# UtkarshSaxena1/CiM_Quantization

Measured on AMD Instinct MI355X. Metric: quantized-MAC/s + fwd+bwd ms per ResNet-20 w3a3 CiM layer, batch 256, higher is better.
Workload: dtype i8+f32; 1 GPU; resnet20_w3a3_all_19_cim_convs_fwd_bwd_sgd; global_batch=256, per_gpu_batch=256, xbar=128, first_layer=w8a8, parallelism=dp1, exchange_segments=1, launch=hip_graph, recompute_psum=False

## Files before the change

### cim_quantization_amd/csrc/cimq_gx5.hip

```cpp
#include "cimq_bwd_dev.h"
#include "cimq_operands.h"

namespace cimq {

__global__ void prep_wg5_kernel(Geo g, const float* __restrict__ w_q, const float* __restrict__ sw_p, int total,
                                v4i* __restrict__ wg5) {
  const WSrc ws{w_q, *sw_p, 0, 0.f, 0.f};
  for (int t = blockIdx.x * blockDim.x + threadIdx.x; t < total; t += gridDim.x * blockDim.x) wg5_item(g, ws, wg5, t);
}

template <int CBN>
__device__ __forceinline__ void gx5_body(int bid, int nblk, const Geo& g, const X5& v, const uint32_t* __restrict__ st,
                                         const v4i* __restrict__ wg5, const Params& pp, const float* __restrict__ sw_p,
                                         const float* __restrict__ sa_p, const float* __restrict__ gout,
                                         const float* __restrict__ x, float* __restrict__ gx,
                                         float* __restrict__ gsa_part) {
  extern __shared__ __attribute__((aligned(16))) uint8_t smem[];
  const int WP = g.W + 2;
  const int PLANE = 6 * WP * 96;
  const int OW5 = 3 * PLANE + 32;
  constexpr int NW5 = 9 * 2 * CBN * 64;
  constexpr int NWI = (NW5 + 511) / 512;
  float* cel = reinterpret_cast<float*>(smem + OW5 + NW5 * 16);
  float* red = cel + 16;
  const int lane = threadIdx.x & 63, wave = threadIdx.x >> 6;
  const int r16 = lane & 15, g4 = lane >> 4;
  const float sw = *sw_p, sa = *sa_p;
  for (int t = threadIdx.x; t < 9; t += blockDim.x) cel[t] = pp.ckj[9 + t];
  if (threadIdx.x < 2) reinterpret_cast<uint4*>(smem + 3 * PLANE)[threadIdx.x] = make_uint4(0u, 0u, 0u, 0u);
  for (int t = threadIdx.x; t < 3 * 6 * 2 * 6; t += blockDim.x) {
    const int q = t % 6, rc = t / 6, side = rc & 1, pr = rc >> 1;
    reinterpret_cast<uint4*>(smem + (size_t)pr * WP * 96 + (side ? (WP - 1) * 96 : 0))[q] = make_uint4(0u, 0u, 0u, 0u);
  }
  __syncthreads();
  const bool std_mask =
      __builtin_amdgcn_ballot_w64(lane < 9 && cel[lane < 9 ? lane : 0] != (float)(1 << (lane / 3))) == 0ull;
  const float scale = sw / 3.f;
  const float inv_sa = 1.f / sa;
  float gpart = 0.f;
  const int cb = wave / v.NPG, pg = wave - cb * v.NPG;
  const int gpr = g.W >> 4;
  const int rl = pg / gpr, iw0 = 16 * (pg - rl * gpr);
  const int c_lo = 16 * cb, c_hi = 16 * cb + 15;
  const int gstride = g.onchw ? g.P : 1;

  const int NG = 6 * g.W * 4;
  for (int mt = bid; mt < v.nmt; mt += nblk) {
    const int b = mt / v.tpi, r0 = (mt - b * v.tpi) * 4;
    v4f acc = v4f{0.f, 0.f, 0.f, 0.f};
    float gvr[2][2][4];
#pragma unroll
    for (int hh = 0; hh < 2; ++hh)
#pragma unroll
      for (int k = 0; k < 2; ++k) {
        const int it = threadIdx.x + k * (int)blockDim.x;
        const int oq = (it & 3) + 4 * hh, rc = it >> 2, col = rc & (g.W - 1), row = rc >> v.lw;
        const int oh = r0 - 1 + row;
#pragma unroll
        for (int e = 0; e < 4; ++e) gvr[hh][k][e] = 0.f;
        if (hh < CBN && it < NG && (unsigned)oh < (unsigned)g.Ho) {
          const int pimg = oh * g.Wo + col;
          const int go = g.onchw ? (b * g.O + 4 * oq) * g.P + pimg : (b * g.P + pimg) * g.O + 4 * oq;
#pragma unroll
          for (int e = 0; e < 4; ++e) gvr[hh][k][e] = gout[go + e * gstride];
        }
      }
    for (int i = 0; i < g.T; ++i)
#pragma unroll
    for (int h = 0; h < 2; ++h) {
      if (h >= CBN) break;
      const int ih2 = i * CBN + h;
      v4i wv[NWI];
#pragma unroll
      for (int u = 0; u < NWI; ++u) {
        const int idx = threadIdx.x + u * 512;
        if (idx < NW5) wv[u] = wg5[ih2 * NW5 + idx];
      }
      uint4 s4r[2];
#pragma unroll
      for (int kk = 0; kk < 2; ++kk) {
        const int it = threadIdx.x + kk * 512;
        const int rc = it >> 2, col = rc & (g.W - 1), row = rc >> v.lw;
        const int oh = r0 - 1 + row;
        s4r[kk] = make_uint4(0u, 0u, 0u, 0u);
        if (it < NG && (unsigned)oh < (unsigned)g.Ho) {
          const int m = b * g.P + oh * g.Wo + col;
          s4r[kk] = *reinterpret_cast<const uint4*>(st + ((i * g.M + m) * g.O + 4 * ((it & 3) + 4 * h)));
        }
      }
      __syncthreads();
#pragma unroll
      for (int u = 0; u < NWI; ++u) {
        const int idx = threadIdx.x + u * 512;
        if (idx < NW5) reinterpret_cast<v4i*>(smem + OW5)[idx] = wv[u];
      }
      auto build = [&](auto stdc) {
        constexpr bool STD = decltype(stdc)::value;
#pragma unroll
        for (int kk = 0; kk < 2; ++kk) {
          const int it = threadIdx.x + kk * (int)blockDim.x;
          if (it >= NG) continue;
          const int oq = (it & 3) + 4 * h, rc = it >> 2, col = rc & (g.W - 1), row = rc >> v.lw;
          const float* gv = gvr[h][kk];
          const uint4 s4 = s4r[kk];
          const uint32_t sv[4] = {s4.x, s4.y, s4.z, s4.w};
          uint8_t* px = smem + (row * WP + col + 1) * 96 + 8 * (oq - 4 * h);
#pragma unroll
          for (int k = 0; k < 3; ++k) {
            float Gv[4];
#pragma unroll
            for (int e = 0; e < 4; ++e) {
              float E;
              if constexpr (STD) {
                E = (float)(__popc(sv[e] & pass_mask_k(k, 3)) << k);
              } else {
                E = 0.f;
#pragma unroll
                for (int j = 0; j < 3; ++j) E += ((sv[e] >> (3 * (k * 3 + j))) & 1u) ? cel[k * 3 + j] : 0.f;
              }
              Gv[e] = gv[e] * E;
            }
            uint32_t ph[2], pm[2], plo[2];
#pragma unroll
            for (int u = 0; u < 2; ++u) split3_pk(Gv[2 * u], Gv[2 * u + 1], ph[u], pm[u], plo[u]);
            *reinterpret_cast<uint2*>(px + 32 * k) = make_uint2(ph[0], ph[1]);
            *reinterpret_cast<uint2*>(px + PLANE + 32 * k) = make_uint2(pm[0], pm[1]);
            *reinterpret_cast<uint2*>(px + 2 * PLANE + 32 * k) = make_uint2(plo[0], plo[1]);
          }
        }
      };
      if (std_mask) build(std::true_type{});
      else build(std::false_type{});
      __syncthreads();
      if (9 * c_hi + 8 < i * g.xbar || 9 * c_lo >= (i + 1) * g.xbar) continue;
      const v4i* wb = reinterpret_cast<const v4i*>(smem + OW5) + cb * 64 + lane;
#pragma unroll
      for (int p = 0; p < 9; ++p) {
        const int kh = p / 3, kw = p - 3 * kh;
        const uint8_t* pa = smem + (size_t)((rl + 2 - kh) * WP + iw0 + r16 + 2 - kw) * 96 + 16 * g4;
#pragma unroll
        for (int s = 0; s < 2; ++s) {
          const v8bf ah = as_v8bf(*reinterpret_cast<const v4i*>(pa + 64 * s));
          const v8bf am = as_v8bf(*reinterpret_cast<const v4i*>(pa + PLANE + 64 * s));
          const v8bf al = as_v8bf(*reinterpret_cast<const v4i*>(pa + 2 * PLANE + 64 * s));
          const v8bf w = as_v8bf(wb[(p * 2 + s) * CBN * 64]);
          acc = __builtin_amdgcn_mfma_f32_16x16x32_bf16(ah, w, acc, 0, 0, 0);
          acc = __builtin_amdgcn_mfma_f32_16x16x32_bf16(am, w, acc, 0, 0, 0);
          acc = __builtin_amdgcn_mfma_f32_16x16x32_bf16(al, w, acc, 0, 0, 0);
        }
      }
    }
    const int ih = r0 + rl, iw = iw0 + 4 * g4;
    const int gi = ((b * g.C + c_lo + r16) * g.H + ih) * g.W + iw;
    const float4 xv4 = *reinterpret_cast<const float4*>(x + gi);
    const float xv[4] = {xv4.x, xv4.y, xv4.z, xv4.w};
    float o4[4];
#pragma unroll
    for (int r = 0; r < 4; ++r) {
      const float gqv = acc[r] * scale;
      const float y1 = xv[r] / sa;
      const float clv = clamp_nan(y1, 0.f, g.lsq_qp);
      const float rr2 = rintf(clv);
      const float rp = (rr2 - clv) + clv;
      const bool pass = (y1 >= 0.f) && (y1 <= g.lsq_qp);
      const float gy = pass ? gqv * sa : 0.f;
      o4[r] = pass ? gqv : 0.f;
      gpart += gqv * rp;
      gpart += -(gy * (y1 * inv_sa));
    }
    *reinterpret_cast<float4*>(gx + gi) = make_float4(o4[0], o4[1], o4[2], o4[3]);
  }
  for (int o = 32; o > 0; o >>= 1) gpart += __shfl_xor(gpart, o);
  __syncthreads();
  if (lane == 0) red[wave] = gpart;
  __syncthreads();
  if (threadIdx.x == 0) {
    float t = 0.f;
    for (int w = 0; w < 8; ++w) t += red[w];
    gsa_part[bid] = t;
  }
}

template <int CBN>
__global__ __attribute__((amdgpu_flat_work_group_size(512, 512), amdgpu_waves_per_eu(4, 8)))
void cim_bwd_gx5_kernel(Geo g, X5 v, const uint32_t* __restrict__ st, const v4i* __restrict__ wg5, Params pp,
                        const float* __restrict__ sw_p, const float* __restrict__ sa_p,
                        const float* __restrict__ gout, const float* __restrict__ x, float* __restrict__ gx,
                        float* __restrict__ gsa_part) {
  gx5_body<CBN>((int)blockIdx.x, (int)gridDim.x, g, v, st, wg5, pp, sw_p, sa_p, gout, x, gx, gsa_part);
}

}
```

### cim_quantization_amd/csrc/cimq_host.h

```cpp
#pragma once
#include <math.h>
#include <stdarg.h>
#include <stdio.h>
#include <string.h>

#include <algorithm>
#include <array>
#include <map>
#include <mutex>
#include <string>

#include "../../include/cimq.h"
#include "cimq_types.h"

namespace cimq {

inline thread_local std::string g_last_error;

inline int fail(int code, const char* fmt, ...) {
  char buf[512];
  va_list ap;
  va_start(ap, fmt);
  vsnprintf(buf, sizeof(buf), fmt, ap);
  va_end(ap);
// ... 538 lines not shown
  return g.input_kind == CIMQ_INPUT_RAW_LSQ && g.NBP == 4 && adc_ok && g.W % 4 == 0 &&
         g.P % 64 == 0 && g.lsq_qp >= 0.f && g.lsq_qp < 255.f && v3_plan(g).ok && (v7_bwd(g) || v7_w44_eval(g)) &&
         !c1_plan(g).ok;
}

struct Plan5 {
  bool ok;
  F5 v;
  size_t lds;
  int nob;
};

inline Plan5 f5_plan_compute(const Geo& g) {
  Plan5 p;
  memset(&p, 0, sizeof(p));
  if (tune("FWD5", 1) == 0) return p;
  if (!fwd_actq_ok(g) || g.mode != ADC_TERNARY || g.variant != VAR_LIBRARY) return p;
  if (g.nbw != 3 || g.nba != 3 || g.bsw != 1 || g.bsa != 1) return p;
  if (g.KH != 3 || g.KW != 3 || g.PH != 1 || g.PW != 1 || g.SH != g.SW || (g.SH != 1 && g.SH != 2)) return p;
  if (g.C % 16 != 0 || g.O % 16 != 0 || g.W % 4 != 0 || g.P % 16 != 0) return p;
  if (g.P >= 128 ? g.P % 128 != 0 : 128 % g.P != 0) return p;
  if (g.M % 128 != 0) return p;
  if (g.Wo % 16 != 0 && 16 % g.Wo != 0) return p;
  F5& v = p.v;
  v.lwo = 0;
  while ((1 << v.lwo) < g.Wo) ++v.lwo;
  if ((1 << v.lwo) != g.Wo) return p;
  v.lwi = 0;
  while ((1 << v.lwi) < g.W) ++v.lwi;
  if ((1 << v.lwi) != g.W) return p;
  if ((long long)g.Nin >= (1LL << 31) || (long long)g.T * g.M * g.O >= (1LL << 31) || (long long)g.M * g.O >= (1LL << 31))
    return p;
  const int PI = std::min(g.P, 128);
  v.IPM = 128 / PI;
  v.R = PI / g.Wo;
  v.RH = (v.R - 1) * g.SH + 3;
  v.WP = g.W + 2;
  v.nmt = g.M / 128;
  v.ntc = 0;
  for (int i = 0; i < g.T; ++i) {
    v.tc0[i] = (unsigned char)v.ntc;
    const int flo = i * g.xbar, fhi = std::min(flo + g.xbar, g.K);
    const int cblo = (flo / 9) / 16, cbhi = ((fhi - 1) / 9) / 16;
    for (int cb = cblo; cb <= cbhi; ++cb) {
      if (v.ntc >= kF5MaxTc) return p;
      v.tcb[v.ntc++] = (unsigned char)cb;
    }
  }
  v.tc0[g.T] = (unsigned char)v.ntc;
  p.nob = (g.OB16 % 2 == 0 && tune("FWD5_NOB2", 1)) ? 2 : 1;
  const size_t fixed = (size_t)p.nob * g.T * 9 * 16 * (16 + 4) + a16((size_t)2 * ((int)g.lsq_qp + 2) * 4) + 16;
  const size_t budget = (size_t)(p.nob == 2 ? tune("FWD5_LDS2_KB", 150) : tune("FWD5_LDS_KB", 80)) * 1024;
  auto need = [&](int tcm, int ncb) {
    return fixed + (size_t)p.nob * tcm * 9 * 1024 + (size_t)v.IPM * v.RH * ncb * v.WP * 48;
  };
  v.ngrp = 0;
  v.tcmax = 0;
  v.NCBP = 0;
  for (int i = 0; i < g.T;) {
    if (v.ngrp >= kF5MaxGrp) return p;
    int e = i + 1;
    auto span = [&](int a, int b) { return v.tcb[v.tc0[b] - 1] - v.tcb[v.tc0[a]] + 1; };
    auto pairs = [&](int a, int b) { return v.tc0[b] - v.tc0[a]; };
    if (need(std::max(v.tcmax, pairs(i, e)), std::max(v.NCBP, span(i, e))) > budget) return p;
    while (e < g.T && need(std::max(v.tcmax, pairs(i, e + 1)), std::max(v.NCBP, span(i, e + 1))) <= budget) ++e;
    const int q = v.ngrp++;
    v.gt0[q] = (unsigned char)i;
    v.gcb0[q] = v.tcb[v.tc0[i]];
    v.gcb1[q] = v.tcb[v.tc0[e] - 1];
    v.gown[q] = (unsigned char)(q == 0 ? v.gcb0[0] : v.gcb1[q - 1] + 1);
    v.tcmax = std::max(v.tcmax, pairs(i, e));
    v.NCBP = std::max(v.NCBP, span(i, e));
    i = e;
  }
  v.gt0[v.ngrp] = (unsigned char)g.T;
  p.lds = need(v.tcmax, v.NCBP);
  p.ok = p.lds <= budget;
  return p;
}
inline Plan5 f5_plan(const Geo& g) { return memo_geo<Plan5, f5_plan_compute>(g); }
inline size_t f5_frag_items(const Geo& g, const Plan5& p) { return p.ok ? (size_t)g.OB16 * p.v.ntc * 9 * 64 : 0; }
inline size_t f5_frag_bytes(const Geo& g) { return f5_frag_items(g, f5_plan(g)) * 16; }

struct PlanG5 {
  bool ok;
  G5 v;
  size_t lds;
  int pairs;
};

inline PlanG5 g5_plan_compute(const Geo& g) {
  PlanG5 p;
  memset(&p, 0, sizeof(p));
  if (tune("GW5", 1) == 0) return p;
  if (!v7_bwd(g) || g.variant != VAR_LIBRARY || g.NBP != 4 || g.nbw != 3 || g.nba != 3 || g.bsa != 1) return p;
  if (g.KH != 3 || g.KW != 3 || g.SH != g.SW || (g.SH != 1 && g.SH != 2) || g.PH != 1 || g.PW != 1 ||
      g.xbar != 128)
    return p;
  if (g.W != g.Wo * g.SH || g.H != g.Ho * g.SH) return p;
  if (g.SH == 2 && tune("GW5_S2", 1) == 0) return p;
  if (g.C % 16 != 0 || g.O % 16 != 0 || g.Wo % 4 != 0) return p;
  if (g.P >= 128 ? g.P % 128 != 0 : (128 % g.P != 0 || g.P % 16 != 0)) return p;
  if (g.M % 128 != 0) return p;
  if (g.T != (9 * g.C + 127) / 128) return p;
  G5& v = p.v;
  v.lwo = 0;
  while ((1 << v.lwo) < g.Wo) ++v.lwo;
  if ((1 << v.lwo) != g.Wo || 128 % g.Wo != 0) return p;
  v.lwi = v.lwo + (g.SH == 2 ? 1 : 0);
  if ((long long)g.Nin >= (1LL << 31)) return p;
  v.IPM = 128 / std::min(g.P, 128);
  v.R = std::min(g.P, 128) / g.Wo;
  v.RH = (v.R - 1) * g.SH + 3;
  v.WP = g.W + 2;
  if ((long long)16 * v.IPM * v.RH * v.WP >= (1LL << 16)) return p;
  if (g.SH == 1 && 16 * v.IPM * v.RH * g.W > 6 * 512) return p;
  v.nmt = g.M / 128;
  p.pairs = (g.C / 16) * g.OB16;
  const int want = std::max(1, tune("GW5_BLOCKS", 512) / p.pairs);
  v.nst = std::max(1, (v.nmt + want - 1) / want);
  v.nchunks = (v.nmt + v.nst - 1) / v.nst;
  p.lds = std::max((size_t)16 * v.IPM * v.RH * v.WP * 8, (size_t)3 * 8 * 64 * 16) + 64 + 4 * 260;
  p.ok = p.lds <= (size_t)80 * 1024;
  return p;
}
inline PlanG5 g5_plan(const Geo& g) { return memo_geo<PlanG5, g5_plan_compute>(g); }

struct PlanX5 {
  bool ok;
  X5 v;
  size_t lds;
  int nblk;
};

inline PlanX5 x5_plan_compute(const Geo& g) {
  PlanX5 p;
  memset(&p, 0, sizeof(p));
  if (tune("GX5", 1) == 0) return p;
  if (!v7_bwd(g) || g.variant != VAR_LIBRARY || g.NBP != 4 || g.nbw != 3 || g.nba != 3 || g.bsw != 1) return p;
  if (g.input_kind != CIMQ_INPUT_RAW_LSQ) return p;
  if (g.KH != 3 || g.KW != 3 || g.SH != 1 || g.SW != 1 || g.PH != 1 || g.PW != 1 || g.xbar != 128) return p;
  const bool c16 = g.C == 16 && g.O == 16 && g.W == 32, c32 = g.C == 32 && g.O == 32 && g.W == 16;
  if (!(c16 || c32) || g.H % 4 != 0 || g.Wo != g.W || g.Ho != g.H || g.T != (9 * g.C + 127) / 128) return p;
  p.v.tpi = g.H / 4;
  p.v.nmt = g.B * p.v.tpi;
  p.v.CBN = g.C / 16;
  p.v.NPG = g.W / 4;
  if (p.v.NPG * p.v.CBN != 8) return p;
  p.v.lw = g.W == 32 ? 5 : 4;
  if (6 * g.W * 4 > 2 * 512) return p;
  if ((long long)g.T * g.M * g.O >= (1LL << 31) || (long long)g.Nin >= (1LL << 31) || (long long)g.M * g.O >= (1LL << 31))
    return p;
  p.nblk = std::min(p.v.nmt, tune("GX5_GRID", 256));
  p.lds = (size_t)3 * 6 * (g.W + 2) * 96 + 32 + (size_t)9 * 2 * p.v.CBN * 1024 + 32 * 4;
  p.ok = p.lds <= (size_t)80 * 1024;
  return p;
}
inline PlanX5 x5_plan(const Geo& g) { return memo_geo<PlanX5, x5_plan_compute>(g); }
inline size_t x5_frag_bytes(const Geo& g) {
  const PlanX5 p = x5_plan(g);
  return p.ok ? (size_t)g.T * p.v.CBN * 9 * 2 * p.v.CBN * 64 * 16 : 0;
}

struct PlanR6 {
  bool ok;
  R6 v;
  size_t lds;
};

inline PlanR6 r6_plan_compute(const Geo& g) {
  PlanR6 p;
  memset(&p, 0, sizeof(p));
  if (!g.recompute || tune("R6", 1) == 0) return p;
  const Plan5 p5 = f5_plan(g);
  if (!p5.ok || !v7_bwd(g) || g.variant != VAR_LIBRARY || g.mode != ADC_TERNARY) return p;
  if (g.input_kind != CIMQ_INPUT_RAW_LSQ || g.nbw != 3 || g.nba != 3 || g.bsw != 1 || g.bsa != 1) return p;
  if (g.KH != 3 || g.KW != 3 || g.SH != 1 || g.SW != 1 || g.PH != 1 || g.PW != 1 || g.xbar != 128) return p;
  if (g.C != kR6C || g.O != kR6C || g.W != kR6W || g.Wo != g.W || g.Ho != g.H || g.H % kR6R != 0) return p;
  if (g.T != kR6T || g.lsq_qp >= 255.f || (long long)g.Nin >= (1LL << 31)) return p;
  if (p5.v.ntc != kR6T || p5.v.tc0[0] != 0 || p5.v.tc0[1] != 1 || p5.v.tc0[2] != 2) return p;
  for (int i = 0; i <= kR6T; ++i) p.v.tc0[i] = p5.v.tc0[i];
  p.v.ntc = p5.v.ntc;
  p.v.nmt = g.H / kR6R;
  p.lds = R6L::LDS;
  p.ok = true;
  return p;
}
inline PlanR6 r6_plan(const Geo& g) { return memo_geo<PlanR6, r6_plan_compute>(g); }
inline size_t r6_frag_bytes(const Geo& g) { return r6_plan(g).ok ? (size_t)kR6WxItems * 16 : 0; }


enum StateFmt {
  ST_NONE,
  ST_PERK,
  ST_V7,
  ST_V7X2,
  ST_PLANES,
  ST_C1,
  ST_DENSE,
};

struct Route {
  int fwd, gx, gw;
  bool actq;
  StateFmt state;
  int cst;
  FwdState fst;
  size_t st_bytes;
  bool codes;
  bool lsq_fused;
  int act_parts;
  int nchunks_bwd;
  int nchunks_ws;
  bool gw_own;
  bool gxw5;
  bool shift_stats;
  bool wgx, wcy, wg5, wx6;
};

inline Route route_compute(const Geo& g) {
  Route r;
  memset(&r, 0, sizeof(r));
  const bool raw = g.input_kind == CIMQ_INPUT_RAW_LSQ, v7b = v7_bwd(g), dense = dense_plan(g);
  r.actq = fwd_actq_ok(g) && (g.onchw || g.inference);
  r.fwd = v3_plan(g).ok ? ((g.onchw && r.actq && f5_plan(g).ok) ? CIMQ_ROUTE_FWD5 : CIMQ_ROUTE_V3)
        : dense         ? CIMQ_ROUTE_DENSE
                        : CIMQ_ROUTE_GENERAL;
  int nchunks, rows;
  gw_chunks(g, &rows, &nchunks);
  const int gen_parts = std::min(cdiv(g.Nin, 256), kLsqParts);
  r.act_parts = gen_parts;
  if (v7b) {
    r.lsq_fused = raw;
    r.nchunks_bwd = r.act_parts = g.B;
    if (g.onchw && !g.inference && r6_plan(g).ok) {
      r.gx = r.gw = CIMQ_ROUTE_R6;
    } else if (c1_plan(g).ok) {
      r.gx = r.gw = CIMQ_ROUTE_C1;
    } else if (v9_plan(g).ok) {
      r.gx = r.gw = CIMQ_ROUTE_FUSED;
    } else {
      const Plan7 p7 = v7_plan(g);
      const PlanX5 px = x5_plan(g);
      const PlanG5 pg = g5_plan(g);
      r.gx = px.ok ? CIMQ_ROUTE_GX5 : CIMQ_ROUTE_V7;
      r.gw = pg.ok ? CIMQ_ROUTE_GW5 : CIMQ_ROUTE_V7;
      r.act_parts = px.ok ? px.nblk : g.B * p7.v.nbands;
      r.nchunks_bwd = pg.ok ? pg.v.nchunks : p7.v.nchunks;
      r.gw_own = g.variant == VAR_LIBRARY;
      r.gxw5 = px.ok && pg.ok && tune("GXW5", 1);
    }
    if (!r.lsq_fused) r.act_parts = gen_parts;
  } else if (dense) {
    r.gx = r.gw = CIMQ_ROUTE_DENSE;
    r.lsq_fused = raw && dense_lsq_parts(g) > 0;
    if (r.lsq_fused) r.act_parts = dense_lsq_parts(g);
    r.nchunks_bwd = cdiv(g.M, dense_rows_per_chunk(g));
  } else {
    r.gx = r.gw = CIMQ_ROUTE_GENERAL;
    r.nchunks_bwd = nchunks;
  }
  r.nchunks_ws = std::max({nchunks, r.nchunks_bwd, r6_plan(g).ok ? g.B : 0});
  r.shift_stats = v7b && g.variant != VAR_LIBRARY;
  const StateFmt fam = dense                 ? ST_DENSE
                     : !v7_plan(g).ok        ? ST_PERK
                     : r.gx == CIMQ_ROUTE_C1 ? ST_C1
                     : g.NBP == 8            ? ST_PLANES
                     : g.nbw == 4            ? ST_V7X2
                                             : ST_V7;
  r.state = r.gx == CIMQ_ROUTE_R6 ? ST_NONE : fam;
  r.cst = (fam == ST_V7 || fam == ST_V7X2) ? g.nbw : (fam == ST_PLANES || fam == ST_C1) ? 8 : 0;
  r.fst = fam == ST_C1 ? FwdState::RECOMPUTE : FwdState::WRITE;
  r.st_bytes = r.state == ST_NONE ? (size_t)0
                                  : std::max({(size_t)g.T * g.nbw * g.M * g.O * (g.NBP == 4 ? 2 : 4),
                                              (size_t)g.T * g.M * g.O * (g.NBP == 4 ? 4 : 24),
                                              dense ? (size_t)g.T * g.M * g.O * 8 : (size_t)0});
  r.codes = r.fwd == CIMQ_ROUTE_FWD5 && r.gw == CIMQ_ROUTE_GW5;
  r.wgx = !v7b;
  r.wcy = v7b;
  r.wg5 = x5_plan(g).ok;
  r.wx6 = r6_plan(g).ok;
  if (g.inference) {
    r.gx = r.gw = CIMQ_ROUTE_NONE;
    r.state = ST_NONE;
    r.st_bytes = 0;
    if (v7_w44_eval(g)) r.cst = 4;
    if (r.cst != 0 && r.fst == FwdState::WRITE) r.fst = FwdState::NONE;
    r.codes = r.lsq_fused = r.gw_own = r.gxw5 = r.wgx = r.wcy = r.wg5 = r.wx6 = false;
  }
  return r;
}
inline Route route_of(const Geo& g) { return memo_geo<Route, route_compute>(g); }

inline FwdMode fwd_mode_of(const Geo& g, const Epi* ep) {
  if (!ep) return g.inference ? FwdMode::INFER : FwdMode::TRAIN;
  return ep->rvw1 ? FwdMode::VIEW : (ep->xq || ep->oq) ? FwdMode::CODES : FwdMode::EPI;
}

inline Geo module_form(Geo g) {
  g.onchw = v3_plan(g).ok ? 1 : 0;
  return g;
}

struct CtxLayout {
  size_t xcode, xhat, alut, wfrag, wf5, wg5, wx6, wgx, wcy, thi, tlo, mlo, mhi, coef, alpha, beta, bsum, ckj, flags, st;
  size_t lsq_scal;
  size_t wbytes;
// ... 250 lines not shown
```

### cim_quantization_amd/csrc/cimq_operands.h

```cpp
#pragma once
#include "cimq_device.h"

namespace cimq {

__device__ inline void pack_word(int8_t (&v)[8], int nbp, uint8_t* dst, long long idx) {
  uint32_t lo = (uint8_t)v[0] | ((uint32_t)(uint8_t)v[1] << 8) | ((uint32_t)(uint8_t)v[2] << 16) |
                ((uint32_t)(uint8_t)v[3] << 24);
  if (nbp == 4) {
    reinterpret_cast<uint32_t*>(dst)[idx] = lo;
  } else {
    uint2 w;
    w.x = lo;
    w.y = (uint8_t)v[4] | ((uint32_t)(uint8_t)v[5] << 8) | ((uint32_t)(uint8_t)v[6] << 16) |
          ((uint32_t)(uint8_t)v[7] << 24);
    reinterpret_cast<uint2*>(dst)[idx] = w;
  }
}

template <bool WB = true>
__device__ inline void act_item(const Geo& g, const float* __restrict__ x, float sa, bool sgn,
                                uint8_t* __restrict__ xcf, uint8_t* __restrict__ xcb, long long idx) {
  float v = x[idx];
  float xq;
  if (g.input_kind == 1) {
// ... 204 lines not shown
      }
      if (NBP == 4) {
        reinterpret_cast<uint4*>(xcf)[t] = make_uint4(f[0][0], f[1][0], f[2][0], f[3][0]);
      } else {
        reinterpret_cast<uint4*>(xcf)[2 * t] = make_uint4(f[0][0], f[0][NW - 1], f[1][0], f[1][NW - 1]);
        reinterpret_cast<uint4*>(xcf)[2 * t + 1] = make_uint4(f[2][0], f[2][NW - 1], f[3][0], f[3][NW - 1]);
      }
    }
  } else {
    for (long long idx = first; idx < g.Nin; idx += step) {
      const int c = min((int)xq[idx], nan_e) * (NBP / 2);
#pragma unroll
      for (int w = 0; w < NW; ++w) dst[idx * NW + w] = lut[c + w];
    }
  }
}

struct WSrc {
  const float* w;
  float sw;
  int raw;
  float qn, qp;
  __device__ float wint(const Geo& g, int o, int f) const {
    const float v = w[(size_t)o * g.K + f];
    if (!raw) return v / sw;
    const float c = clamp_nan(v / sw, qn, qp);
    const float wq = round_pass_value(c) * sw;
    return wq / sw;
  }
};

__device__ inline float wslice(const Geo& g, const WSrc& ws, int f, int n) {
  const int k = n / g.Opad, o = n - k * g.Opad;
  if (f >= g.K || o >= g.O || k >= g.nbw) return 0.f;
  return slice_signed(ws.wint(g, o, f), k, g.bsw);
}

__device__ inline void wfrag_item(const Geo& g, const WSrc& ws, v4i* __restrict__ wfrag, int t) {
  const int lane = t % WAVE;
  int r = t / WAVE;
  const int nb = r % g.NBLK;
  r /= g.NBLK;
  const int ks = r % g.KS;
  const int i = r / g.KS;
  const int flo = i * g.xbar, fhi = min(flo + g.xbar, g.K);
  const int n = nb * 16 + (lane & 15);
  uint32_t wd[4] = {0, 0, 0, 0};
#pragma unroll
  for (int e = 0; e < 16; ++e) {
    const int f = flo + ks * 64 + 16 * (lane >> 4) + e;
    int v = 0;
    if (f < fhi) v = clamp_i8(wslice(g, ws, f, n));
    wd[e >> 2] |= ((uint32_t)(uint8_t)(int8_t)v) << (8 * (e & 3));
  }
  v4i o;
  o.x = (int)wd[0]; o.y = (int)wd[1]; o.z = (int)wd[2]; o.w = (int)wd[3];
  wfrag[t] = o;
}

__device__ inline void wgx_item(const Geo& g, const WSrc& ws, v4i* __restrict__ wgx, int t) {
  const int lane = t % WAVE;
  int r = t / WAVE;
  const int s = r % g.NKS;
  r /= g.NKS;
  const int fb = r % g.FBT;
  const int i = r / g.FBT;
  const int flo = i * g.xbar, fhi = min(flo + g.xbar, g.K);
  const int f = flo + fb * 16 + (lane & 15);
  uint32_t wd[4] = {0, 0, 0, 0};
#pragma unroll
  for (int e = 0; e < 8; ++e) {
    const int kb = 2 * s + (e >> 2);
    const int kap = kb * 16 + 4 * (lane >> 4) + (e & 3);
    float v = 0.f;
    if (f < fhi && kb < g.NBLK) v = (float)to_i8_wrap(wslice(g, ws, f, kap));
    const uint32_t h = bf16_bits(v);
    wd[e >> 1] |= h << (16 * (e & 1));
  }
  v4i o;
  o.x = (int)wd[0]; o.y = (int)wd[1]; o.z = (int)wd[2]; o.w = (int)wd[3];
  wgx[t] = o;
}

__device__ inline void wcy_item(const Geo& g, const WSrc& ws, int ncpbt, v4i* __restrict__ wcy, int t) {
  const int lane = t % WAVE;
  int r = t / WAVE;
  const int s = r % g.NKS;
  r /= g.NKS;
  const int cb = r % ncpbt;
  const int i = r / ncpbt;
  const int flo = i * g.xbar, fhi = min(flo + g.xbar, g.K);
  const int rho = lane & 15;
  const int cp = ((flo / g.KW) / 4 + cb) * 4 + (rho >> 2), kw = rho & 3;
  const int c = cp / g.KH, kh = cp - c * g.KH;
  const int f = c * g.KHW + kh * g.KW + kw;
  const bool ok = kw < g.KW && c < g.C && f >= flo && f < fhi;
  uint32_t wd[4] = {0, 0, 0, 0};
#pragma unroll
  for (int e = 0; e < 8; ++e) {
    const int kb = 2 * s + (e >> 2);
    const int kap = kb * 16 + 4 * (lane >> 4) + (e & 3);
    float v = 0.f;
    if (ok && kb < g.NBLK) v = (float)to_i8_wrap(wslice(g, ws, f, kap));
    wd[e >> 1] |= (uint32_t)bf16_bits(v) << (16 * (e & 1));
  }
  v4i o;
  o.x = (int)wd[0]; o.y = (int)wd[1]; o.z = (int)wd[2]; o.w = (int)wd[3];
  wcy[t] = o;
}

template <typename WS>
__device__ inline void wf5_item(const Geo& g, const F5W& v, const WS& ws, v4i* __restrict__ wf5, int t) {
  const int lane = t & 63;
  int r = t >> 6;
  const int k = r % 3;
  r /= 3;
  const int s = r % 3;
  r /= 3;
  const int tc = r % v.ntc;
  const int ob = r / v.ntc;
  int i = 0;
  while (v.tc0[i + 1] <= tc) ++i;
  const int flo = i * g.xbar, fhi = min(flo + g.xbar, g.K);
  const int p = 4 * s + (lane >> 4);
  const int n = k * g.Opad + ob * 16 + (lane & 15);
  uint32_t wd[4] = {0, 0, 0, 0};
  if (p < 9) {
#pragma unroll
    for (int e = 0; e < 16; ++e) {
      const int c = v.tcb[tc] * 16 + e;
      const int f = c * 9 + p;
      int val = 0;
      if (c < g.C && f >= flo && f < fhi) val = clamp_i8(wslice(g, ws, f, n));
      wd[e >> 2] |= ((uint32_t)(uint8_t)(int8_t)val) << (8 * (e & 3));
    }
  }
  v4i o;
  o.x = (int)wd[0]; o.y = (int)wd[1]; o.z = (int)wd[2]; o.w = (int)wd[3];
  wf5[t] = o;
}

template <typename WS>
__device__ inline void wg5_item(const Geo& g, const WS& ws, v4i* __restrict__ wg5, int t) {
  const int CBN = g.C / 16;
  const int lane = t & 63;
  int r = t >> 6;
  const int cb = r % CBN;
  r /= CBN;
  const int s = r & 1;
  r >>= 1;
  const int p = r % 9;
  r /= 9;
  const int h = r % CBN, i = r / CBN;
  const int c = 16 * cb + (lane & 15);
  const int f = c * 9 + p;
  const int flo = i * g.xbar, fhi = min(flo + g.xbar, g.K);
  const bool ok = c < g.C && f >= flo && f < fhi;
  uint32_t wd[4] = {0, 0, 0, 0};
#pragma unroll
  for (int e = 0; e < 8; ++e) {
    const int kap = 32 * s + 8 * (lane >> 4) + e;
    const int k = kap >> 4, o = 16 * h + (kap & 15);
    float val = 0.f;
    if (ok && k < g.nbw) val = (float)to_i8_wrap(wslice(g, ws, f, k * g.Opad + o));
    wd[e >> 1] |= (uint32_t)bf16_bits(val) << (16 * (e & 1));
  }
  v4i q;
  q.x = (int)wd[0]; q.y = (int)wd[1]; q.z = (int)wd[2]; q.w = (int)wd[3];
  wg5[t] = q;
}

template <typename WS>
__device__ inline void wx6_item(const Geo& g, const WS& ws, v4i* __restrict__ wx6, int t) {
  const int lane = t & 63;
  const int r = t >> 6;
  const int s = r % kR6KSG, p = r / kR6KSG;
  const int c = lane & 15;
  const int f = c * 9 + p;
  uint32_t wd[4] = {0, 0, 0, 0};
#pragma unroll
  for (int e = 0; e < 8; ++e) {
    const int kap = 32 * s + 8 * (lane >> 4) + e;
    const int i = kap / kR6KO, rem = kap - i * kR6KO, k = rem >> 4, o = rem & 15;
    float val = 0.f;
    if (c < g.C && i < g.T && f >= i * g.xbar && f < min((i + 1) * g.xbar, g.K) && k < g.nbw)
      val = (float)to_i8_wrap(wslice(g, ws, f, k * g.Opad + o));
    wd[e >> 1] |= (uint32_t)bf16_bits(val) << (16 * (e & 1));
  }
  v4i q;
  q.x = (int)wd[0]; q.y = (int)wd[1]; q.z = (int)wd[2]; q.w = (int)wd[3];
  wx6[t] = q;
}

__device__ inline int first_true_ternary_hi(int lo, int hi, float sw, float sa, float a) {
  int L = lo, R = hi + 1;
  while (L < R) {
    int mid = L + ((R - L) >> 1);
    float q = rintf(u_of(mid, sw, sa) / a);
    if (q >= 1.f) R = mid; else L = mid + 1;
  }
  return L;
}
__device__ inline int last_true_ternary_lo(int lo, int hi, float sw, float sa, float a) {
  int L = lo - 1, R = hi;
  while (L < R) {
    int mid = L + ((R - L + 1) >> 1);
    float q = rintf(u_of(mid, sw, sa) / a);
    if (q <= -1.f) L = mid; else R = mid - 1;
  }
  return L;
}

struct ASrc {
  const float* a;
  int raw;
  float scale, qp_al;
  __device__ float get(int e) const {
    if (!raw) return a[e];
    const float t = a[e] / scale;
    return clamp_nan(round_pass_value(t), 1.f, qp_al) * scale;
  }
};

__device__ inline bool scales_ok(float sw, float sa) {
  return (sw * sa > 0.f) && isfinite(sw * sa) && isfinite(sw) && isfinite(sa);
}

__device__ inline bool params_item(const Geo& g, const ASrc& as, float sw, float sa,
                                   const int8_t* __restrict__ bmask, const Params& pp, int t,
                                   const float* __restrict__ beta = nullptr) {
  const int npar = g.T * g.nba * g.nbw * g.Opad;
  const int nkj = g.nbw * g.nba;
  if (t >= npar + nkj) {
    const int o = t - npar - nkj;
    float b = 0.f;
    if (beta != nullptr && o < g.O)
      for (int i = 0; i < g.T; ++i)
        for (int k = 0; k < g.nbw; ++k)
          for (int j = 0; j < g.nba; ++j)
            b += beta[((i * g.nbw + k) * g.nba + j) * g.O + o] * (float)bmask[k * g.nba + j];
    pp.bsum[o] = b;
    return false;
  }
  if (t >= npar) {
    const int kj = t - npar, k = kj / g.nba, j = kj - k * g.nba;
    const float mk = (float)bmask[k * g.nba + j];
    pp.ckj[kj] = mk;
    pp.ckj[nkj + kj] = mk * pow2f(-g.bsa * j);
    pp.ckj[2 * nkj + kj] = mk * pow2f(-g.bsw * k);
    return false;
  }
  int r = t;
  const int o = r % g.Opad; r /= g.Opad;
  const int k = r % g.nbw; r /= g.nbw;
  const int j = r % g.nba;
  const int i = r / g.nba;
  const float mk = (float)bmask[k * g.nba + j];
  float a = 1.f;
  if (has_alpha(g) && as.a != nullptr && o < g.O)
    a = as.get(((i * g.nbw + k) * g.nba + j) * g.O + o);
  pp.alpha[t] = a;
  pp.beta[t] = (beta != nullptr && o < g.O) ? beta[((i * g.nbw + k) * g.nba + j) * g.O + o] : 0.f;
  pp.coef[t] = a * mk;
  const int lo = -g.psmax - 1, hi = g.psmax + 1;
  bool literal = false;
  int thi = hi + 1, tlo = lo - 1, mlo = hi + 1, mhi = lo - 1;
  if (g.mode == ADC_SIGN || g.mode == ADC_TERNARY) {
    if (!(scales_ok(sw, sa) && a > 0.f && isfinite(a))) literal = true;
  }
  const bool sf = shift_fast(g);
  const float be = pp.beta[t];
  if (g.variant != VAR_LIBRARY && !sf) literal = true;
  if (sf && !isfinite(be)) literal = true;
  if (!literal) {
    if (sf) {
      int L = lo, R = hi + 1;
      while (L < R) {
        const int mid = L + ((R - L) >> 1);
        if (rintf(psb_value(g, mid, sw, sa, a, be)) >= 1.f) R = mid; else L = mid + 1;
      }
      thi = L;
      L = lo - 1; R = hi;
      while (L < R) {
        const int mid = L + ((R - L + 1) >> 1);
        if (rintf(psb_value(g, mid, sw, sa, a, be)) <= -1.f) L = mid; else R = mid - 1;
      }
      tlo = L;
    } else if (g.mode == ADC_TERNARY) {
      thi = first_true_ternary_hi(lo, hi, sw, sa, a);
      tlo = last_true_ternary_lo(lo, hi, sw, sa, a);
    }
    {
      int L = lo, R = hi + 1;
      while (L < R) {
        int mid = L + ((R - L) >> 1);
        float b = sf ? psb_value(g, mid, sw, sa, a, be) : psb_literal(mid, g.mode, sw, sa, a);
        if (b > g.thr_lo) R = mid; else L = mid + 1;
      }
      mlo = L;
      L = lo - 1; R = hi;
      while (L < R) {
        int mid = L + ((R - L + 1) >> 1);
        float b = sf ? psb_value(g, mid, sw, sa, a, be) : psb_literal(mid, g.mode, sw, sa, a);
        if (b < g.thr_hi) L = mid; else R = mid - 1;
      }
      mhi = L;
    }
  }
  pp.thi[t] = thi;
  pp.tlo[t] = tlo;
// ... 7 lines not shown
```

### cim_quantization_amd/csrc/cimq_types.h

```cpp
#pragma once

#include <hip/hip_runtime.h>
#include <stdint.h>

namespace cimq {

#define WAVE 64

typedef int v4i __attribute__((ext_vector_type(4)));
typedef float v4f __attribute__((ext_vector_type(4)));
typedef __bf16 v8bf __attribute__((ext_vector_type(8)));

enum AdcMode { ADC_FP = 0, ADC_SIGN = 1, ADC_TERNARY = 2, ADC_MULTI = 3 };
enum AdcVariant { VAR_LIBRARY = 0, VAR_STOCHASTIC = 1, VAR_SHIFT_ROUND = 2, VAR_SHIFT_SIGN = 3 };

struct Geo {
  int B, C, H, W, O, KH, KW, SH, SW, PH, PW, Ho, Wo;
  int P, M, K, KHW, HW;
  int xbar, T, KS, KTP;
  int FBT;
  int nbw, nba, bsw, bsa, NBP;
  int Opad, OB16, NBLK, NKS;
  int mode;
  float qn, qp, thr_hi, thr_lo;
// ... 42 lines not shown
  return ResView{(int)(w0 & 0xffffu), (int)(w0 >> 16), (int)(w1 >> 30) + 1, (int)(w1 & 0x7fffu), (int)((w1 >> 15) & 0x7fffu)};
}
inline void set_res_view(Epi* ep, int c0, int cr, int s, int h, int w) {
  ep->rvw0 = (uint32_t)c0 | (uint32_t)cr << 16;
  ep->rvw1 = (uint32_t)h | (uint32_t)w << 15 | (uint32_t)(s - 1) << 30;
}

enum class FwdMode : int {
  TRAIN,
  INFER,
  EPI,
  CODES,
  VIEW,
};
constexpr bool has_epi(FwdMode m) { return m >= FwdMode::EPI; }
constexpr bool has_codes(FwdMode m) { return m >= FwdMode::CODES; }
constexpr bool has_view(FwdMode m) { return m >= FwdMode::VIEW; }
constexpr bool writes_state(FwdMode m) { return m == FwdMode::TRAIN; }
enum class FwdState : int { WRITE, RECOMPUTE, NONE };

__host__ __device__ inline int pidx(const Geo& g, int i, int j, int k, int o) {
  return ((i * g.nba + j) * g.nbw + k) * g.Opad + o;
}

__host__ __device__ inline bool shift_fast(const Geo& g) {
  return g.variant == VAR_SHIFT_ROUND && g.mode == ADC_TERNARY && !g.ps_int8 && g.qp == 1.f && g.qn == -1.f &&
         g.psmax <= 2048;
}

struct V3 {
  int lw;
  int RH;
  int obm;
  int WP;
  int RI, nbands;
  int RHB;
  int NPB;
  int fwd_res;
  int nmt;
  int NCG;
  int NCBT;
  int CB;
  int NT;
  int pf;
};

struct V7 {
  int lw;
  int NCPBT;
  int SWD;
  int NSEG;
  int NRS;
  int RSLOT;
  int NPART;
  int lwin, lcin;
  int RB;
  int nbands;
  int FBX;
  int NSLOT;
  int CPITCH;
  int nstage;
  int nchunks;
  int whole;
  int CPL;
  int NTL;
  int GSH;
  int KWP;
};

struct V9 {
  int lw;
  int R;
  int nsteps;
  int SWD, NSEG;
  int RSLOT;
  int NCPBT;
  int lcin;
  int NCG;
  int CPITCH;
  int KWP;
  int PROWS;
  int NGRP;
  int gwl;
  int nitems;
  unsigned o_ring, o_cel, o_red, o_plane, o_gwl, o_gal, o_st, o_g, lds;
};

struct VC1 {
  int lw;
  int R;
  int nsteps;
  int RH, WP;
  int SWD, NSEG, RSLOT;
  int NCPBT;
  int lcin;
  unsigned o_xp, o_hp, o_ptab, o_prm, o_cel, o_g, o_ring, o_gal, o_red, o_e, o_wk, o_wc, lds;
};

constexpr int kF5MaxTc = 8;
constexpr int kF5MaxGrp = 4;

struct F5 {
  int lwo;
  int lwi;
  int codes;
  int IPM;
  int R, RH, WP;
  int NCBP;
  int nmt;
  int ntc;
  int ngrp;
  int tcmax;
  int tc0[kF5MaxTc + 1];
  int tcb[kF5MaxTc];
  int gt0[kF5MaxGrp + 1];
  int gcb0[kF5MaxGrp], gcb1[kF5MaxGrp];
  int gown[kF5MaxGrp];
};

struct F5W {
  int ntc;
  unsigned char tc0[kF5MaxTc + 1];
  unsigned char tcb[kF5MaxTc];
};
inline F5W f5w_of(const F5& v) {
  F5W w;
  w.ntc = v.ntc;
  for (int i = 0; i <= kF5MaxTc; ++i) w.tc0[i] = v.tc0[i];
  for (int i = 0; i < kF5MaxTc; ++i) w.tcb[i] = v.tcb[i];
  return w;
}

constexpr int kZeroCode = 259;

struct G5 {
  int lwo;
  int lwi;
  int codes;
  int IPM;
  int R, RH, WP;
  int nmt;
  int nst;
  int nchunks;
};

struct X5 {
  int nmt;
  int tpi;
  int CBN;
  int NPG;
  int lw;
};

struct R6 {
  int tc0[3];
  int ntc;
  int nmt;
};

constexpr int kR6C = 16, kR6W = 32, kR6R = 4, kR6T = 2;
constexpr int kR6KO = 3 * kR6C;
constexpr int kR6NK = kR6T * kR6KO;
constexpr int kR6KSG = kR6NK / 32;
constexpr int kR6WxItems = 9 * kR6KSG * 64;

struct R6L {
  static constexpr int RP = kR6R + 2, WP = kR6W + 2;
  static constexpr int GPX = kR6NK * 2 + 16;
  static constexpr int GROW = WP * GPX;
  static constexpr int GPL = kR6R * GROW;
  static constexpr int EXP = 36;
  static constexpr int O_XP = 0;
  static constexpr int O_XH = O_XP + RP * WP * 48;
  static constexpr int O_GP = O_XH + kR6C * RP * WP * 8;
  static constexpr int O_CA = O_GP + 3 * GPL;
  static constexpr int O_WX = O_CA + 2 * kR6C * kR6W * 4;
  static constexpr int O_PR = O_WX + kR6WxItems * 16;
  static constexpr int O_AL = O_PR + kR6T * 9 * 16 * 16;
  static constexpr int O_CE = O_AL + 260 * 8;
  static constexpr int LDS = O_CE + 32 * 4;
};
static_assert(R6L::LDS <= 160 * 1024, "r6 LDS budget");
static_assert(9 * 8 * 64 * 16 <= 3 * R6L::GPL, "r6 gw reduction buffer");
static_assert(2 * kR6T * 9 * 8 * 16 * 4 <= 3 * R6L::GPL, "r6 grad_alpha reduction buffer");

constexpr int kCalFlag = 300;
constexpr uint32_t kCodesMagic = 0xC0DE5EEDu;

constexpr int kActLutMax = 256;

}
```

Before: 4593 billion MAC/s.

## Exploit sparse crossbar tile in gx5 via shifted kw accumulators and compact weights

Restructures the input-gradient MFMA loop so each kh row loads one activation slab and accumulates the three kw taps into separate accumulators, then combines them with lane shuffles and an LDS exchange at tile edges. This removes the per-kw activation LDS reads. For the crossbar tile that covers only a few channels, it packs those channels' kw taps into one compact 16-column weight operand, so that tile needs fewer MFMAs and fewer weight loads. In exchange it adds more accumulator registers, shuffles, an extra barrier for CBN==1, and hardcoded geometry assumptions (xbar 128, 16/32 channels).

Result: no change. 4617 billion MAC/s (median of 6 runs) (+0.5%).

```diff
diff --git a/cim_quantization_amd/csrc/cimq_gx5.hip b/cim_quantization_amd/csrc/cimq_gx5.hip
--- a/cim_quantization_amd/csrc/cimq_gx5.hip
+++ b/cim_quantization_amd/csrc/cimq_gx5.hip
@@ -20,9 +20,11 @@
   const int PLANE = 6 * WP * 96;
   const int OW5 = 3 * PLANE + 32;
   constexpr int NW5 = 9 * 2 * CBN * 64;
-  constexpr int NWI = (NW5 + 511) / 512;
+  constexpr int NWI = ((9 + 3) * 2 * 64 + 511) / 512;
+  static_assert(x5_compact(0).tile == 1 && (CBN == 1 || x5_compact(1).tile == 2), "block cb: full tile cb, compact cb + 1");
   float* cel = reinterpret_cast<float*>(smem + OW5 + NW5 * 16);
   float* red = cel + 16;
+  float* xch = red + 16;
   const int lane = threadIdx.x & 63, wave = threadIdx.x >> 6;
   const int r16 = lane & 15, g4 = lane >> 4;
   const float sw = *sw_p, sa = *sa_p;
@@ -42,12 +44,15 @@
   const int gpr = g.W >> 4;
   const int rl = pg / gpr, iw0 = 16 * (pg - rl * gpr);
   const int c_lo = 16 * cb, c_hi = 16 * cb + 15;
+  const X5Compact cpt = CBN == 2 && cb == 1 ? x5_compact(1) : x5_compact(0);
   const int gstride = g.onchw ? g.P : 1;
 
   const int NG = 6 * g.W * 4;
   for (int mt = bid; mt < v.nmt; mt += nblk) {
     const int b = mt / v.tpi, r0 = (mt - b * v.tpi) * 4;
-    v4f acc = v4f{0.f, 0.f, 0.f, 0.f};
+    v4f U[3], V = v4f{0.f, 0.f, 0.f, 0.f};
+#pragma unroll
+    for (int kw = 0; kw < 3; ++kw) U[kw] = v4f{0.f, 0.f, 0.f, 0.f};
     float gvr[2][2][4];
 #pragma unroll
     for (int hh = 0; hh < 2; ++hh)
@@ -70,11 +75,16 @@
     for (int h = 0; h < 2; ++h) {
       if (h >= CBN) break;
       const int ih2 = i * CBN + h;
+      const int nfull = i < CBN ? 9 * 2 * 64 : 0, nw = nfull + (i > 0 ? 3 * 2 * 64 : 0);
+      auto widx = [&](int j) {
+        const int jj = j < nfull ? j : j - nfull, cbs = j < nfull ? i : i - 1;
+        return ((jj >> 6) * CBN + cbs) * 64 + (jj & 63);
+      };
       v4i wv[NWI];
 #pragma unroll
       for (int u = 0; u < NWI; ++u) {
-        const int idx = threadIdx.x + u * 512;
-        if (idx < NW5) wv[u] = wg5[ih2 * NW5 + idx];
+        const int j = threadIdx.x + u * 512;
+        if (j < nw) wv[u] = wg5[ih2 * NW5 + widx(j)];
       }
       uint4 s4r[2];
 #pragma unroll
@@ -91,8 +101,8 @@
       __syncthreads();
 #pragma unroll
       for (int u = 0; u < NWI; ++u) {
-        const int idx = threadIdx.x + u * 512;
-        if (idx < NW5) reinterpret_cast<v4i*>(smem + OW5)[idx] = wv[u];
+        const int j = threadIdx.x + u * 512;
+        if (j < nw) reinterpret_cast<v4i*>(smem + OW5)[widx(j)] = wv[u];
       }
       auto build = [&](auto stdc) {
         constexpr bool STD = decltype(stdc)::value;
@@ -134,22 +144,63 @@
       __syncthreads();
       if (9 * c_hi + 8 < i * g.xbar || 9 * c_lo >= (i + 1) * g.xbar) continue;
       const v4i* wb = reinterpret_cast<const v4i*>(smem + OW5) + cb * 64 + lane;
-#pragma unroll
-      for (int p = 0; p < 9; ++p) {
-        const int kh = p / 3, kw = p - 3 * kh;
-        const uint8_t* pa = smem + (size_t)((rl + 2 - kh) * WP + iw0 + r16 + 2 - kw) * 96 + 16 * g4;
+      const bool compact = i == cpt.tile;
+#pragma unroll
+      for (int kh = 0; kh < 3; ++kh) {
+        const uint8_t* pa = smem + (size_t)((rl + 2 - kh) * WP + iw0 + r16 + 1) * 96 + 16 * g4;
 #pragma unroll
         for (int s = 0; s < 2; ++s) {
           const v8bf ah = as_v8bf(*reinterpret_cast<const v4i*>(pa + 64 * s));
           const v8bf am = as_v8bf(*reinterpret_cast<const v4i*>(pa + PLANE + 64 * s));
           const v8bf al = as_v8bf(*reinterpret_cast<const v4i*>(pa + 2 * PLANE + 64 * s));
-          const v8bf w = as_v8bf(wb[(p * 2 + s) * CBN * 64]);
-          acc = __builtin_amdgcn_mfma_f32_16x16x32_bf16(ah, w, acc, 0, 0, 0);
-          acc = __builtin_amdgcn_mfma_f32_16x16x32_bf16(am, w, acc, 0, 0, 0);
-          acc = __builtin_amdgcn_mfma_f32_16x16x32_bf16(al, w, acc, 0, 0, 0);
-        }
-      }
-    }
+          if (compact) {
+            const v8bf w = as_v8bf(wb[(kh * 2 + s) * CBN * 64]);
+            V = __builtin_amdgcn_mfma_f32_16x16x32_bf16(ah, w, V, 0, 0, 0);
+            V = __builtin_amdgcn_mfma_f32_16x16x32_bf16(am, w, V, 0, 0, 0);
+            V = __builtin_amdgcn_mfma_f32_16x16x32_bf16(al, w, V, 0, 0, 0);
+          } else {
+            v8bf w[3];
+#pragma unroll
+            for (int kw = 0; kw < 3; ++kw) w[kw] = as_v8bf(wb[((3 * kh + kw) * 2 + s) * CBN * 64]);
+#pragma unroll
+            for (int kw = 0; kw < 3; ++kw) U[kw] = __builtin_amdgcn_mfma_f32_16x16x32_bf16(ah, w[kw], U[kw], 0, 0, 0);
+#pragma unroll
+            for (int kw = 0; kw < 3; ++kw) U[kw] = __builtin_amdgcn_mfma_f32_16x16x32_bf16(am, w[kw], U[kw], 0, 0, 0);
+#pragma unroll
+            for (int kw = 0; kw < 3; ++kw) U[kw] = __builtin_amdgcn_mfma_f32_16x16x32_bf16(al, w[kw], U[kw], 0, 0, 0);
+          }
+        }
+      }
+    }
+    {
+      const int cf = cpt.c_first - c_lo;
+      const bool live = r16 >= cf;
+      const int src = (lane & 48) | (live ? 3 * (r16 - cf) : 0);
+#pragma unroll
+      for (int kw = 0; kw < 3; ++kw)
+#pragma unroll
+        for (int r = 0; r < 4; ++r) {
+          const float t = __shfl(V[r], src + kw);
+          U[kw][r] += live ? t : 0.f;
+        }
+    }
+    float e0 = __shfl(U[0][0], (lane + 16) & 63);
+    float e2 = __shfl(U[2][3], (lane - 16) & 63);
+    if constexpr (CBN == 1) {
+      if (g4 == 0) xch[wave * 32 + r16] = U[0][0];
+      if (g4 == 3) xch[wave * 32 + 16 + r16] = U[2][3];
+      __syncthreads();
+      if (g4 == 3) e0 = iw0 == 0 ? xch[(wave + 1) * 32 + r16] : 0.f;
+      if (g4 == 0) e2 = iw0 != 0 ? xch[(wave - 1) * 32 + 16 + r16] : 0.f;
+    } else {
+      if (g4 == 3) e0 = 0.f;
+      if (g4 == 0) e2 = 0.f;
+    }
+    v4f acc;
+    acc[0] = (U[1][0] + U[0][1]) + e2;
+    acc[1] = (U[1][1] + U[0][2]) + U[2][0];
+    acc[2] = (U[1][2] + U[0][3]) + U[2][1];
+    acc[3] = (U[1][3] + e0) + U[2][2];
     const int ih = r0 + rl, iw = iw0 + 4 * g4;
     const int gi = ((b * g.C + c_lo + r16) * g.H + ih) * g.W + iw;
     const float4 xv4 = *reinterpret_cast<const float4*>(x + gi);
diff --git a/cim_quantization_amd/csrc/cimq_host.h b/cim_quantization_amd/csrc/cimq_host.h
--- a/cim_quantization_amd/csrc/cimq_host.h
+++ b/cim_quantization_amd/csrc/cimq_host.h
@@ -714,7 +714,7 @@
   if ((long long)g.T * g.M * g.O >= (1LL << 31) || (long long)g.Nin >= (1LL << 31) || (long long)g.M * g.O >= (1LL << 31))
     return p;
   p.nblk = std::min(p.v.nmt, tune("GX5_GRID", 256));
-  p.lds = (size_t)3 * 6 * (g.W + 2) * 96 + 32 + (size_t)9 * 2 * p.v.CBN * 1024 + 32 * 4;
+  p.lds = (size_t)3 * 6 * (g.W + 2) * 96 + 32 + (size_t)9 * 2 * p.v.CBN * 1024 + 32 * 4 + 8 * 32 * 4;
   p.ok = p.lds <= (size_t)80 * 1024;
   return p;
 }
diff --git a/cim_quantization_amd/csrc/cimq_operands.h b/cim_quantization_amd/csrc/cimq_operands.h
--- a/cim_quantization_amd/csrc/cimq_operands.h
+++ b/cim_quantization_amd/csrc/cimq_operands.h
@@ -380,10 +380,19 @@
   const int p = r % 9;
   r /= 9;
   const int h = r % CBN, i = r / CBN;
-  const int c = 16 * cb + (lane & 15);
-  const int f = c * 9 + p;
   const int flo = i * g.xbar, fhi = min(flo + g.xbar, g.K);
-  const bool ok = c < g.C && f >= flo && f < fhi;
+  const X5Compact cc = x5_compact(cb);
+  int f;
+  bool ok;
+  if (i == cc.tile) {
+    const int n = lane & 15, c = cc.c_first + n / 3;
+    f = c * 9 + 3 * p + (n - 3 * (n / 3));
+    ok = p < 3 && n < 3 * cc.nch && f >= flo && f < fhi;
+  } else {
+    const int c = 16 * cb + (lane & 15);
+    f = c * 9 + p;
+    ok = c < g.C && f >= flo && f < fhi;
+  }
   uint32_t wd[4] = {0, 0, 0, 0};
 #pragma unroll
   for (int e = 0; e < 8; ++e) {
diff --git a/cim_quantization_amd/csrc/cimq_types.h b/cim_quantization_amd/csrc/cimq_types.h
--- a/cim_quantization_amd/csrc/cimq_types.h
+++ b/cim_quantization_amd/csrc/cimq_types.h
@@ -218,6 +218,18 @@
   int lw;
 };
 
+struct X5Compact {
+  int tile, c_first, nch;
+};
+constexpr X5Compact x5_compact(int cb) {
+  const int tile = (144 * cb + 143) / 128;
+  const int f0 = 128 * tile > 144 * cb ? 128 * tile : 144 * cb;
+  return X5Compact{tile, f0 / 9, 16 * cb + 16 - f0 / 9};
+}
+static_assert(3 * x5_compact(0).nch <= 16 && 3 * x5_compact(1).nch <= 16, "compact columns must fit one MFMA operand");
+static_assert(x5_compact(0).tile == 1 && x5_compact(0).c_first == 14 && x5_compact(1).tile == 2 &&
+              x5_compact(1).c_first == 28, "the sparse pairs of 16 / 32 input channels at xbar 128");
+
 struct R6 {
   int tc0[3];
   int ntc;
```
